# Jittor/InstanceSegmentation-jittor

Hardware: AMD Instinct MI355X
Metric: images/sec (Yolact R50-FPN 550x550, bs=8 per GPU, fp32) (higher is better)
Workload: dtype f32; 1 GPU; Yolact R50-FPN 550x550 bs=8/GPU random weights: uint8 upload + FastBaseTransform on the device + backbone+FPN+protonet+heads+Detect(fast-NMS)+550x550 mask assembly (BASELINE configs[1]); global_batch=8, parallelism=batch-sharded x1, RCCL all-gather of detections

## Files before the change

### include/isegmi.h

```cpp
#ifndef ISEGMI_H
#define ISEGMI_H
#include <stdint.h>
#ifdef __cplusplus
extern "C" {
#endif
#pragma GCC visibility push(default)

#define ISEGMI_ABI_VERSION 1

int isegmi_version(void);
const char* isegmi_last_error(void);

int isegmi_device_count(int* n);
int isegmi_set_device(int device_id);
int isegmi_malloc(void** d_ptr, int64_t bytes);
int isegmi_free(void* d_ptr);
int isegmi_malloc_host(void** h_ptr, int64_t bytes);
int isegmi_free_host(void* h_ptr);
int isegmi_h2d(void* d_dst, const void* h_src, int64_t bytes);
int isegmi_d2h(void* h_dst, const void* d_src, int64_t bytes);
int isegmi_memset(void* d_ptr, int value, int64_t bytes);
int isegmi_sync(void);
int isegmi_box_calibrate(double ms_per_leg, double* mfma_f32_tflops, double* mfma_f16_tflops, double* hbm_copy_gbs);

typedef struct isegmi_conv_desc {
    int32_t N, H, W, Cin;
    int32_t Cout, R, S, stride, pad;
    int32_t act;
    int32_t tile;
    int32_t out_div;
    int64_t out_img_stride;
    int64_t out_pix_stride;
} isegmi_conv_desc;

int isegmi_conv_out_hw(const isegmi_conv_desc* d, int32_t* Ho, int32_t* Wo);
int isegmi_conv_split_qualifies(const isegmi_conv_desc* d);
int isegmi_conv_packed_floats(const isegmi_conv_desc* d, int64_t* n);
int isegmi_pack_conv_weights(const isegmi_conv_desc* d, const float* h_w_krsc, float* h_packed);
int isegmi_op_conv2d(const isegmi_conv_desc* d, const float* d_in, const float* d_wpacked,
                     const float* d_scale, const float* d_shift, const float* d_residual,
                     float* d_out, void* stream);
int isegmi_op_conv2d_group(int n, const isegmi_conv_desc* descs, const float* const* d_in, const float* const* d_w, const float* const* d_scale,
                           const float* const* d_shift, const float* const* d_res, float* const* d_out, void* stream);

int isegmi_conv_grouped_packed_floats(const isegmi_conv_desc* d, int groups, int64_t* n);
int isegmi_pack_conv_weights_grouped(const isegmi_conv_desc* d, int groups, const float* h_w, float* h_packed);
int isegmi_op_conv2d_grouped(const isegmi_conv_desc* d, int groups, const float* d_in, const float* d_wpacked,
                             const float* d_scale, const float* d_shift, const float* d_residual,
                             float* d_out, void* stream);

int isegmi_conv_packed_halfs(const isegmi_conv_desc* d, int64_t* n);
int isegmi_pack_conv_weights_f16(const isegmi_conv_desc* d, const float* h_w_krsc, uint16_t* h_packed);
int isegmi_op_conv2d_f16(const isegmi_conv_desc* d, const void* d_in, const void* d_wpacked,
                         const float* d_scale, const float* d_shift, const void* d_residual, void* d_out,
                         int out_f32, void* stream);
typedef struct isegmi_bottleneck_desc {
    int32_t N, H, W, Cin, Cmid;
    int32_t flags;
} isegmi_bottleneck_desc;
int isegmi_op_bottleneck_f16(const isegmi_bottleneck_desc* d, const void* d_x, const void* d_w1, const float* d_s1, const float* d_b1,
                             const void* d_w2, const float* d_s2, const float* d_b2, const void* d_w3, const float* d_s3,
                             const float* d_b3, void* d_out, void* stream);
int isegmi_op_bottleneck_ds_f16(const isegmi_bottleneck_desc* d, const void* d_x, const void* d_w1, const float* d_s1, const float* d_b1,
                                const void* d_w2, const float* d_s2, const float* d_b2, const void* d_w3, const float* d_s3,
                                const float* d_b3, const void* d_wd, const float* d_sd, const float* d_bd, void* d_out, void* stream);
int isegmi_op_conv1x1_up2x_add_f16(const isegmi_conv_desc* d, const void* d_in, const void* d_wpacked, const float* d_scale, const float* d_shift,
                                   const void* d_coarse, int Hc, int Wc, void* d_out, void* stream);
int isegmi_op_conv3x3_head_f16(const isegmi_conv_desc* d, const void* d_in, const void* d_wpacked, const float* d_scale, const float* d_shift,
                               const void* d_w2packed, const float* d_scale2, const float* d_shift2, int cout2, float* d_out2, int* fused, void* stream);
int isegmi_op_pad_c3_to_f16_halo(const float* d_in_nhwc3, int N, int H, int W, void* d_out, void* stream);
int isegmi_op_stem_pool_f16(int N, int H, int W, const void* d_halo, const void* d_w, const float* d_scale, const float* d_shift, void* d_out,
                            int flags, void* stream);

int isegmi_set_f16_mfma_shape(int shape);
int isegmi_get_f16_mfma_shape(int* shape);

// ... 405 lines not shown
```

### instancesegmentation-jittor_amd/csrc/conv_mfma.hip

```cpp
#include <type_traits>
#include "../../include/isegmi.h"
#include "common.h"
#include "conv_korder.h"
#include "detmath.h"

#ifndef CONV_F32_RES_AUX
#define CONV_F32_RES_AUX 0
#endif

namespace isegmi {

typedef float f32x16 __attribute__((ext_vector_type(16)));

struct ConvK {
    const float* in;
    const float* w;
    const float* scale;
    const float* shift;
    const float* res;
    float* out;
    int N, H, W, Cin, Cout, R, S, stride, pad, Ho, Wo, M;
    int nchunks, cin_chunks;
    int kgroup;
    int64_t wrow;
// ... 221 lines not shown
                    acc[a][b] = __builtin_amdgcn_mfma_f32_32x32x2f32(fa[a].w, fb[b].w, acc[a][b], 0, 0, 0);
                }
        }
    };

    int cur = 0;
    for (int t = 0; t + 1 < p.nchunks; ++t) {
        load_chunk(t + 1);
        __builtin_amdgcn_sched_barrier(0);
        compute(cur);
        __builtin_amdgcn_sched_barrier(0);
        store_chunk(cur ^ 1);
        __syncthreads();
        cur ^= 1;
    }
    compute(cur);

#pragma unroll
    for (int a = 0; a < TM; ++a) {
#pragma unroll
        for (int b = 0; b < TN; ++b) {
            const int co = n0 + (wn * TN + b) * 32 + lr;
            const bool cok = co < p.Cout;
            const float sc = (cok && p.scale) ? p.scale[co] : 1.0f;
            const float sh = (cok && p.shift) ? p.shift[co] : 0.0f;
            Epi ep;
            epi_begin(p, m0 + (wm * TM + a) * 32 + 4 * lh, co, ep);
            epi_finish(p, acc[a][b], sc, sh, ep);
            __builtin_amdgcn_sched_barrier(0);
        }
    }
}

template <int RING, bool EARLY>
__device__ __forceinline__ void conv_v2_body(const ConvK& p, float* smem, const int bid, const int nwg) {
    constexpr int BM = 64, BN = 64;
    constexpr int STAGE = (BM + BN) * LDS_ROW;
    const int tid = threadIdx.x;
    const int lane = tid & 63, wave = __builtin_amdgcn_readfirstlane(tid >> 6);
    const int wm = wave >> 1, wn = wave & 1;
    const int q8 = nwg >> 3, r8 = nwg & 7, xcd = bid & 7;
    const int logical = (xcd < r8 ? xcd * (q8 + 1) : r8 * (q8 + 1) + (xcd - r8) * q8) + (bid >> 3);
    int mt, nt;
    conv_tile_of(p, logical, mt, nt);
    const int m0 = p.m_begin + mt * BM, n0 = nt * BN;

    const int lrow = tid >> 2, g = tid & 3;
    int hi0, wi0;
    unsigned abase;
    {
        const int m = m0 + lrow;
        if (m >= p.M) { hi0 = -(1 << 28); wi0 = 0; abase = 0; }
        else if (p.R * p.S == 1 && p.stride == 1 && p.pad == 0) {
            hi0 = 0; wi0 = 0;
            abase = ((unsigned)m * (unsigned)p.Cin + (unsigned)(g * 8)) * 4u;
        } else {
            const int hw = p.Ho * p.Wo;
            const int n = m / hw, rem = m - n * hw;
            const int ho = rem / p.Wo, wo = rem - ho * p.Wo;
            hi0 = ho * p.stride - p.pad; wi0 = wo * p.stride - p.pad;
            abase = ((unsigned)((n * p.H + hi0) * p.W + wi0) * (unsigned)p.Cin + (unsigned)(g * 8)) * 4u;
        }
    }
    const unsigned wbase = ((unsigned)(n0 + lrow) * (unsigned)p.wrow + (unsigned)(g * 8)) * 4u;
    constexpr unsigned OOB = 0x80000000u;
    typedef unsigned int u32x4 __attribute__((ext_vector_type(4)));
    auto make_rsrc = [](const void* ptr, unsigned bytes) {
        const unsigned long long a = (unsigned long long)ptr;
// ... 18 lines not shown
        asm volatile("buffer_load_dwordx4 %0, %1, %2, %3 offen" : "=v"(rb[slot][0]) : "v"(wbase), "s"(rsb), "s"(soffb) : "memory");
        asm volatile("buffer_load_dwordx4 %0, %1, %2, %3 offen offset:16" : "=v"(rb[slot][1]) : "v"(wbase), "s"(rsb), "s"(soffb) : "memory");
        ++chunk;
        soffa += 128u;
        if (conv_k_next(kr, ks, kc, kg, glen, p.R, p.S, p.kgroup, p.cin_chunks)) {
            soffa = (unsigned)kg * 128u;
            int tr = __builtin_amdgcn_readfirstlane(kr), ts = __builtin_amdgcn_readfirstlane(ks);
            asm volatile("" : "+s"(tr), "+s"(ts));
            const unsigned inb = (unsigned)((unsigned)(hi0 + tr) < (unsigned)p.H) & (unsigned)((unsigned)(wi0 + ts) < (unsigned)p.W);
            const unsigned tapv = abase + (unsigned)((tr * p.W + ts) * p.Cin) * 4u;
            avoff = inb ? tapv : OOB;
        }
    };
    typedef __attribute__((address_space(3))) void* lds_ptr;
    const unsigned lds_wr_addr = (unsigned)(uintptr_t)(lds_ptr)(smem + lrow * LDS_ROW + g * 8);
    auto store_chunk = [&](int slot, int stage, auto pending) {
        asm volatile("s_waitcnt vmcnt(%4)" : "+v"(ra[slot][0]), "+v"(ra[slot][1]), "+v"(rb[slot][0]), "+v"(rb[slot][1]) : "n"(decltype(pending)::value) : "memory");
        const unsigned wa = lds_wr_addr + (unsigned)(stage * STAGE * 4);
        asm volatile("ds_write2_b32 %0, %1, %2 offset1:1" :: "v"(wa), "v"(ra[slot][0].x), "v"(ra[slot][0].z) : "memory");
        asm volatile("ds_write2_b32 %0, %1, %2 offset0:2 offset1:3" :: "v"(wa), "v"(ra[slot][1].x), "v"(ra[slot][1].z) : "memory");
        asm volatile("ds_write2_b32 %0, %1, %2 offset0:4 offset1:5" :: "v"(wa), "v"(ra[slot][0].y), "v"(ra[slot][0].w) : "memory");
        asm volatile("ds_write2_b32 %0, %1, %2 offset0:6 offset1:7" :: "v"(wa), "v"(ra[slot][1].y), "v"(ra[slot][1].w) : "memory");
        asm volatile("ds_write_b128 %0, %1 offset:%2" :: "v"(wa), "v"(rb[slot][0]), "n"(BM * LDS_ROW * 4) : "memory");
        asm volatile("ds_write_b128 %0, %1 offset:%2" :: "v"(wa), "v"(rb[slot][1]), "n"(BM * LDS_ROW * 4 + 16) : "memory");
        asm volatile("s_waitcnt lgkmcnt(0)" ::: "memory");
    };

    f32x16 acc;
#pragma unroll
    for (int e = 0; e < 16; ++e) acc[e] = 0.0f;
    const int lr = lane & 31, lh = lane >> 5;
    const float* const lds_a = smem + (wm * 32 + lr) * LDS_ROW + lh * 4;
    const float* const lds_b = smem + BM * LDS_ROW + (wn * 32 + lr) * LDS_ROW + lh * 4;
    float4 fa[2], fb[2];
    auto read_frags = [&](int set, int stage, int gg) {
        fa[set] = *(const float4*)(lds_a + stage * STAGE + gg * 8);
        fb[set] = *(const float4*)(lds_b + stage * STAGE + gg * 8);
    };
    auto mma4 = [&](int set) {
        acc = __builtin_amdgcn_mfma_f32_32x32x2f32(fa[set].x, fb[set].x, acc, 0, 0, 0);
        acc = __builtin_amdgcn_mfma_f32_32x32x2f32(fa[set].y, fb[set].y, acc, 0, 0, 0);
        acc = __builtin_amdgcn_mfma_f32_32x32x2f32(fa[set].z, fb[set].z, acc, 0, 0, 0);
        acc = __builtin_amdgcn_mfma_f32_32x32x2f32(fa[set].w, fb[set].w, acc, 0, 0, 0);
    };
    auto compute = [&](int stage) {
#pragma unroll
        for (int gg = 0; gg < 4; ++gg) {
            if (gg < 3) read_frags((gg + 1) & 1, stage, gg + 1);
            mma4(gg & 1);
        }
    };
    typedef std::integral_constant<int, 4 * (RING - 1)> Steady;
    typedef std::integral_constant<int, 4 * (RING - 2) < 0 ? 0 : 4 * (RING - 2)> Early;
    static_assert(RING % 2 == 0, "the LDS stage of an unrolled position is its parity");

#pragma unroll
    for (int i = 0; i < RING; ++i) load_chunk(i);
    store_chunk(0, 0, Steady());
    __syncthreads();
    const int last = p.nchunks - 1;
    for (int t0 = 0; t0 < last; t0 += RING) {
#pragma unroll
        for (int j = 0; j < RING; ++j) {
            if (t0 + j >= last) break;
            const int cur = j & 1;
            read_frags(0, cur, 0);
            if (EARLY) store_chunk((j + 1) % RING, cur ^ 1, Early());
            load_chunk(j);
            __builtin_amdgcn_sched_barrier(0);
            compute(cur);
            __builtin_amdgcn_sched_barrier(0);
            if (!EARLY) store_chunk((j + 1) % RING, cur ^ 1, Steady());
            __syncthreads();
        }
    }
    const int cur = last & 1;
    const int co = n0 + wn * 32 + lr;
    const bool cok = co < p.Cout;
    Epi ep;
    epi_begin(p, m0 + wm * 32 + 4 * lh, co, ep);
    const float sc = (cok && p.scale) ? p.scale[co] : 1.0f;
    const float sh = (cok && p.shift) ? p.shift[co] : 0.0f;
    __builtin_amdgcn_sched_barrier(0);
    read_frags(0, cur, 0);
    compute(cur);
    __builtin_amdgcn_sched_barrier(0);
    asm volatile("s_waitcnt vmcnt(0)" ::: "memory");
#pragma unroll
    for (int i = 0; i < RING; ++i) asm volatile("" :: "v"(ra[i][0]), "v"(ra[i][1]), "v"(rb[i][0]), "v"(rb[i][1]));
    epi_finish(p, acc, sc, sh, ep);
}

template <int RING, bool EARLY>
__global__ __launch_bounds__(256, 4) void conv_mfma_v2_kernel(const ConvK p) {
    extern __shared__ __attribute__((aligned(16))) float smem[];
    conv_v2_body<RING, EARLY>(p, smem, (int)blockIdx.x, (int)gridDim.x);
}

typedef float f32x4 __attribute__((ext_vector_type(4)));

#ifndef EXPERIMENT_HALF_B
#define EXPERIMENT_HALF_B 0
#endif
#ifndef EXPERIMENT_NO_LOADS
#define EXPERIMENT_NO_LOADS 0
#endif
#ifndef EXPERIMENT_MODE
#define EXPERIMENT_MODE 0
#endif
template <int RING, bool LW, int WN = 1, int KS = 1>
__device__ __forceinline__ void conv_mfma16_body(const ConvK& p, float* smem16, const int bid, const int nwg) {
    static_assert(WN == 1 || !LW, "the loader-wave variant runs one tile per wave");
    static_assert(KS == 1 || (!LW && WN == 1), "split-K runs KS plain 32 x 32 sets");
    constexpr int BM = 32, BN = 32 * WN;
    constexpr int ROW = 34;
    constexpr int STAGE = (BM + BN) * ROW;
    constexpr int NST = LW ? 3 : 2;
    float* const smem_block = smem16;
    const int kset = KS > 1 ? __builtin_amdgcn_readfirstlane((int)(threadIdx.x >> 8)) : 0;
    if (KS > 1) smem16 += kset * NST * STAGE;
    const int count = KS > 1 ? (p.nchunks + KS - 1) / KS : p.nchunks;
    const int c_begin = KS > 1 ? min(kset * count, p.nchunks) : 0;
    const int c_end = KS > 1 ? min(c_begin + count, p.nchunks) : p.nchunks;

    const int tid = threadIdx.x & 255;
    const bool loader = LW && __builtin_amdgcn_readfirstlane((int)(threadIdx.x >> 8)) != 0;
    const int lane = tid & 63, wave = __builtin_amdgcn_readfirstlane(tid >> 6);
    const int wm = wave >> 1, wn = wave & 1;
    const int q8 = nwg >> 3, r8 = nwg & 7, xcd = bid & 7;
// ... 243 lines not shown
            for (int e = 0; e < 4; ++e) {
                float y = fmaf(acc[t][e], sc, sh);
                if (p.act == 4) {
                    y = y > 0.0f ? y : y * 0.1f;
                    yv[e] = y + rv[e];
                    continue;
                }
                y = y + rv[e];
                yv[e] = p.act == 3 ? (y > 0.0f ? y : y * 0.1f) : y;
            }
            if (p.act == 2) {
#pragma unroll
                for (int e = 0; e < 4; ++e) yv[e] = dm_tanh(yv[e]);
            }
        }
#pragma unroll
        for (int e = 0; e < 4; ++e) __builtin_amdgcn_raw_buffer_store_b32(__builtin_bit_cast(unsigned, yv[e]), rs_out, ooff[e], 0, 0);
    }
}

template <int RING, bool LW, int WN = 1>
__global__ __launch_bounds__(LW ? 512 : 256) void conv_mfma16_kernel(const ConvK p) {
    constexpr int STAGE16 = (32 + 32 * WN) * 34;
    __shared__ __attribute__((aligned(16))) float smem16[(LW ? 3 : 2) * STAGE16];
    conv_mfma16_body<RING, LW, WN>(p, smem16, (int)blockIdx.x, (int)gridDim.x);
}

template <int KS>
__global__ __launch_bounds__(256 * KS) void conv_mfma16_split_kernel(const ConvK p) {
    extern __shared__ __attribute__((aligned(16))) float smem_split[];
    conv_mfma16_body<4, false, 1, KS>(p, smem_split, (int)blockIdx.x, (int)gridDim.x);
}

template <int RING>
__global__ __launch_bounds__(256, 4) void conv_hybrid_kernel(const ConvK pm, const ConvK pt, const int nmain) {
    extern __shared__ __attribute__((aligned(16))) float smem[];
    if ((int)blockIdx.x < nmain) conv_v2_body<RING, false>(pm, smem, (int)blockIdx.x, nmain);
    else conv_mfma16_body<4, false, 1>(pt, smem, (int)blockIdx.x - nmain, (int)gridDim.x - nmain);
}

constexpr int CONV_GROUP_MAX = 10;
struct ConvGroupK {
    int n;
    int blk0[CONV_GROUP_MAX + 1];
    int kind[CONV_GROUP_MAX];
    ConvK k[CONV_GROUP_MAX];
};
static_assert(sizeof(ConvGroupK) <= 4096, "kernel arguments");
template <int RING>
__global__ __launch_bounds__(256, 4) void conv_group_kernel(const ConvGroupK g) {
    extern __shared__ __attribute__((aligned(16))) float smem[];
    int i = 0;
    while (i + 1 < g.n && (int)blockIdx.x >= g.blk0[i + 1]) ++i;
    const int bid = (int)blockIdx.x - g.blk0[i], nwg = g.blk0[i + 1] - g.blk0[i];
    if (g.kind[i] == 0) conv_v2_body<RING, false>(g.k[i], smem, bid, nwg);
    else conv_mfma16_body<4, false, 1>(g.k[i], smem, bid, nwg);
}

static bool is_stem(const isegmi_conv_desc* d) { return d->Cin == 4 && d->R == 7 && d->S == 7; }
static int cout_pad(const isegmi_conv_desc* d) { return cdiv(d->Cout, 128) * 128; }
static int n_chunks(const isegmi_conv_desc* d) { return is_stem(d) ? 7 : d->R * d->S * (d->Cin / 32); }

static int check_desc(const isegmi_conv_desc* d) {
    ARG_CHECK(d != nullptr, "null desc");
    ARG_CHECK(d->N > 0 && d->H > 0 && d->W > 0 && d->Cout > 0 && d->R > 0 && d->S > 0 && d->stride > 0 && d->pad >= 0,
              "non-positive conv geometry");
    ARG_CHECK(is_stem(d) || (d->Cin > 0 && d->Cin % 32 == 0), "Cin must be a multiple of 32 (or the Cin=4 7x7 stem)");
    ARG_CHECK(d->H + 2 * d->pad >= d->R && d->W + 2 * d->pad >= d->S, "kernel larger than padded input");
    ARG_CHECK(d->act >= 0 && d->act <= 4, "act");
    ARG_CHECK(d->tile >= 0 && d->tile <= 15, "tile");
    return ISEGMI_OK;
}

static void conv_set_band(ConvK& k, const int bn, const int blocks_per_cu, const int64_t in_touched) {
    static int legacy = -1;
    if (legacy < 0) { const char* e = getenv("ISEGMI_CONV_BAND"); legacy = (e && atoi(e) == 0) ? 1 : 0; }
    if (legacy) { k.nband = (int64_t)k.w_bytes > (int64_t)k.in_bytes ? 1 : k.ntiles; return; }
    const double A = (double)in_touched, B = (double)k.nchunks * 128.0 * bn * k.ntiles;
    const double l2_keep = 2.5e6;
    const double slots = 32.0 * blocks_per_cu;
    const double tiles_xcd = (double)k.mtiles * k.ntiles / 8.0;
    const double rounds = tiles_xcd / slots > 1.0 ? tiles_xcd / slots : 1.0;
    double best = 0;
    int best_bw = k.ntiles;
    for (int nb = 1; nb <= k.ntiles; nb *= 2) {
        const int bw = cdiv(k.ntiles, nb), nbands = cdiv(k.ntiles, bw);
        const double band_b = B / nbands;
        double a, b;
// ... 43 lines not shown
    k.in = in; k.w = w; k.scale = scale; k.shift = shift; k.res = res; k.out = out;
    k.N = d->N; k.H = d->H; k.W = d->W; k.Cin = d->Cin; k.Cout = d->Cout; k.R = d->R; k.S = d->S;
    k.stride = d->stride; k.pad = d->pad;
    k.Ho = (d->H + 2 * d->pad - d->R) / d->stride + 1;
    k.Wo = (d->W + 2 * d->pad - d->S) / d->stride + 1;
    const int64_t M64 = (int64_t)d->N * k.Ho * k.Wo;
    ARG_CHECK(M64 < (1ll << 31) - 256, "too many output pixels");
    k.M = (int)M64;
    k.nchunks = n_chunks(d);
    k.cin_chunks = is_stem(d) ? 1 : d->Cin / 32;
    k.kgroup = conv_kgroup(d->R, d->S, k.cin_chunks, is_stem(d));
    k.wrow = (int64_t)k.nchunks * 32;
    const int64_t in_bytes = (int64_t)d->N * d->H * d->W * d->Cin * 4;
    ARG_CHECK(in_bytes < (1ll << 31), "conv input must be < 2 GiB (32-bit buffer offsets)");
    k.in_bytes = (unsigned)in_bytes;
    k.w_bytes = (unsigned)((int64_t)cout_pad(d) * k.wrow * 4);
    k.in_touched = (d->R == 1 && d->S == 1 && d->stride > 1) ? in_bytes / ((int64_t)d->stride * d->stride) : in_bytes;
    k.m_begin = 0;
    k.act = d->act;
    k.out_div = d->out_div > 0 ? d->out_div : k.Ho * k.Wo;
    k.out_pix_stride = d->out_pix_stride > 0 ? d->out_pix_stride : d->Cout;
    k.out_img_stride = d->out_img_stride > 0 ? d->out_img_stride : (int64_t)k.out_div * k.out_pix_stride;
    k.contiguous = (k.out_img_stride == (int64_t)k.out_div * k.out_pix_stride) ? 1 : 0;
    const int64_t n_img = (k.M + k.out_div - 1) / k.out_div;
    const int64_t out_extent = ((n_img - 1) * k.out_img_stride + (int64_t)(k.out_div - 1) * k.out_pix_stride + d->Cout) * 4;
    ARG_CHECK(out_extent < (1ll << 31), "conv output span must be < 2 GiB (32-bit buffer offsets)");
    k.out_bytes = (unsigned)out_extent;
    k.res_bytes = (unsigned)((int64_t)k.M * d->Cout * 4);
    ARG_CHECK(res == nullptr || (int64_t)k.M * d->Cout * 4 < (1ll << 31), "residual must be < 2 GiB");
    k.mtiles = 0; k.ntiles = 0; k.nband = 0;
    return ISEGMI_OK;
}

static bool conv_hybrid_on() {
    static int on = -1;
    if (on < 0) { const char* e = getenv("ISEGMI_CONV_HYBRID"); on = (e && atoi(e) == 0) ? 0 : 1; }
    return on != 0;
}

int conv2d_launch(const isegmi_conv_desc* d, const float* in, const float* w, const float* scale, const float* shift,
                  const float* res, float* out, hipStream_t st) {
    ConvK k;
    const int rc_fill = conv_fill(d, in, w, scale, shift, res, out, k);
    if (rc_fill) return rc_fill;
    int tile = d->tile;
    if (tile == 0) {
        const int64_t t64 = (int64_t)cdiv(k.M, 64) * cdiv(d->Cout, 64);
        const int nck = k.nchunks;
        const int ncu = device_cu_count();
        const int v2 = nck >= 72 ? 12 : 10;
        if (is_stem(d)) tile = 3;
        else if (t64 <= 176) tile = 5;
        else if (nck <= 2 && d->Cout > 32) tile = v2;
        else if (d->Cout <= 32 || t64 <= 480) tile = 4;
        else if (t64 >= 513 && t64 % ncu != 0 && (t64 % ncu) * 100 <= t64 * 15 && conv_hybrid_on()) tile = 13;
        else if (t64 <= 512) tile = v2;
        else if (t64 <= 640) tile = nck >= 32 ? 6 : 4;
        else if (t64 <= 1024) tile = v2;
        else if (t64 <= 1100) tile = nck >= 32 ? 6 : 4;
        else tile = v2;
    }
    if (tile >= 4 && is_stem(d)) tile = 3;
    if (tile == 13 || tile == 14) {
        const int nt64 = cdiv(d->Cout, 64);
        const int64_t mt64 = cdiv(k.M, 64);
        const int ncu = device_cu_count();
        int64_t main_mt = (mt64 * nt64 / ncu) * ncu / nt64;
        if (main_mt * 64 > k.M) main_mt = k.M / 64;
        if (main_mt <= 0 || main_mt >= mt64) {
            tile = tile == 13 ? 10 : 12;
        } else {
            ConvK km = k, kt = k;
            km.mtiles = (int)main_mt; km.ntiles = nt64;
            kt.m_begin = (int)(main_mt * 64);
            kt.mtiles = cdiv(k.M - kt.m_begin, 32); kt.ntiles = cdiv(d->Cout, 32);
            const int64_t in_tail = (int64_t)((double)k.in_touched * (k.M - kt.m_begin) / k.M);
            conv_set_band(km, 64, 4, k.in_touched - in_tail);
            conv_set_band(kt, 32, 4, in_tail);
            const int nmain = km.mtiles * km.ntiles, ntail = kt.mtiles * kt.ntiles;
            const size_t lds = 2 * (size_t)(64 + 64) * LDS_ROW * sizeof(float);
            if (tile == 13) hipLaunchKernelGGL((conv_hybrid_kernel<2>), dim3((unsigned)(nmain + ntail)), dim3(256), lds, st, km, kt, nmain);
            else hipLaunchKernelGGL((conv_hybrid_kernel<4>), dim3((unsigned)(nmain + ntail)), dim3(256), lds, st, km, kt, nmain);
            HIP_TRY(hipGetLastError());
            return ISEGMI_OK;
        }
    }
    if (tile == 15) {
        ARG_CHECK(!is_stem(d), "split-K: not for the stem");
        constexpr int KS = 4;
        k.mtiles = cdiv(k.M, 32);
        k.ntiles = cdiv(d->Cout, 32);
        conv_set_band(k, 32, 1, k.in_touched);
        const size_t lds = (size_t)KS * 2 * (32 + 32) * 34 * sizeof(float);
        LDS_LIMIT_ONCE((int)lds, conv_mfma16_split_kernel<KS>);
        hipLaunchKernelGGL((conv_mfma16_split_kernel<KS>), dim3((unsigned)(k.mtiles * k.ntiles)), dim3(256 * KS), lds, st, k);
        HIP_TRY(hipGetLastError());
        return ISEGMI_OK;
    }
    if (tile >= 7) {
        ARG_CHECK(tile != 8 && tile != 11, "tiles 8 / 11 (ring of 3) were dropped: the LDS stage of an unrolled position is its parity");
        k.mtiles = cdiv(k.M, 64);
        k.ntiles = cdiv(d->Cout, 64);
        const size_t lds = 2 * (size_t)(64 + 64) * LDS_ROW * sizeof(float);
        conv_set_band(k, 64, 4, k.in_touched);
        const dim3 g7((unsigned)(k.mtiles * k.ntiles));
        if (tile == 7) hipLaunchKernelGGL((conv_mfma_v2_kernel<2, true>), g7, dim3(256), lds, st, k);
        else if (tile == 9) hipLaunchKernelGGL((conv_mfma_v2_kernel<4, true>), g7, dim3(256), lds, st, k);
        else if (tile == 10) hipLaunchKernelGGL((conv_mfma_v2_kernel<2, false>), g7, dim3(256), lds, st, k);
        else hipLaunchKernelGGL((conv_mfma_v2_kernel<4, false>), g7, dim3(256), lds, st, k);
        HIP_TRY(hipGetLastError());
        return ISEGMI_OK;
    }
    if (tile >= 4) {
        k.mtiles = cdiv(k.M, 32);
        k.ntiles = cdiv(d->Cout, tile == 6 ? 64 : 32);
        conv_set_band(k, tile == 6 ? 64 : 32, tile == 4 ? 8 : 4, k.in_touched);
        const dim3 g16((unsigned)(k.mtiles * k.ntiles));
        if (tile == 5) hipLaunchKernelGGL((conv_mfma16_kernel<8, true>), g16, dim3(512), 0, st, k);
        else if (tile == 6) hipLaunchKernelGGL((conv_mfma16_kernel<4, false, 2>), g16, dim3(256), 0, st, k);
        else hipLaunchKernelGGL((conv_mfma16_kernel<4, false>), g16, dim3(256), 0, st, k);
        HIP_TRY(hipGetLastError());
        return ISEGMI_OK;
    }
    switch (tile) {
        case 1: return launch<128, 128, 2, 2>(d, k, st);
        case 2: return launch<128, 64, 2, 2>(d, k, st);
        default: return launch<64, 64, 2, 2>(d, k, st);
    }
}

int conv2d_group_launch(int n, const isegmi_conv_desc* const* d, const float* const* in, const float* const* w, const float* const* scale,
                        const float* const* shift, const float* const* res, float* const* out, hipStream_t st) {
    ARG_CHECK(n >= 1 && n <= CONV_GROUP_MAX && d && in && w && out, "conv group: 1..10 members");
    ConvGroupK g;
    ConvK ks[CONV_GROUP_MAX];
    int64_t t64[CONV_GROUP_MAX], total64 = 0;
    for (int i = 0; i < n; ++i) {
        ARG_CHECK(d[i] && !is_stem(d[i]) && d[i]->tile == 0, "conv group: no stem, no forced tile");
        ARG_CHECK(in[i] && w[i] && out[i], "conv group: a member's input, weights or output pointer is NULL");
        const int rc = conv_fill(d[i], in[i], w[i], scale ? scale[i] : nullptr, shift ? shift[i] : nullptr, res ? res[i] : nullptr, out[i], ks[i]);
        if (rc) return rc;
        t64[i] = (int64_t)cdiv(ks[i].M, 64) * cdiv(d[i]->Cout, 64);
        total64 += t64[i];
    }
    int order[CONV_GROUP_MAX], kind[CONV_GROUP_MAX];
    int ring = 2;
    for (int i = 0; i < n; ++i) {
        order[i] = i;
        kind[i] = (total64 > 480 && t64[i] >= 256 && d[i]->Cout > 32) ? 0 : 1;
        if (kind[i] == 0 && ks[i].nchunks >= 72) ring = 4;
    }
    for (int a = 1; a < n; ++a)
        for (int b = a; b > 0; --b) {
            const int x = order[b - 1], y = order[b];
            const bool swap = kind[y] < kind[x] || (kind[y] == kind[x] && t64[y] > t64[x]);
            if (!swap) break;
            order[b - 1] = y; order[b] = x;
        }
    g.n = n;
    g.blk0[0] = 0;
    for (int j = 0; j < n; ++j) {
        const int i = order[j];
        ConvK& k = ks[i];
        const int bt = kind[i] == 0 ? 64 : 32;
        k.mtiles = cdiv(k.M, bt);
        k.ntiles = cdiv(d[i]->Cout, bt);
        conv_set_band(k, bt, kind[i] == 0 ? 4 : 8, k.in_touched);
        const int64_t blocks = (int64_t)k.mtiles * k.ntiles;
        ARG_CHECK(g.blk0[j] + blocks < (1ll << 30), "conv group: too many tiles");
        g.k[j] = k;
        g.kind[j] = kind[i];
        g.blk0[j + 1] = g.blk0[j] + (int)blocks;
    }
    const size_t lds = 2 * (size_t)(64 + 64) * LDS_ROW * sizeof(float);
    if (ring == 4) hipLaunchKernelGGL((conv_group_kernel<4>), dim3((unsigned)g.blk0[n]), dim3(256), lds, st, g);
    else hipLaunchKernelGGL((conv_group_kernel<2>), dim3((unsigned)g.blk0[n]), dim3(256), lds, st, g);
    HIP_TRY(hipGetLastError());
    return ISEGMI_OK;
}

}

using namespace isegmi;

extern "C" int isegmi_op_conv2d_group(int n, const isegmi_conv_desc* descs, const float* const* d_in, const float* const* d_w, const float* const* d_scale,
                                      const float* const* d_shift, const float* const* d_res, float* const* d_out, void* stream) {
    ARG_CHECK(n >= 1 && n <= CONV_GROUP_MAX && descs, "conv group: 1..10 members");
    const isegmi_conv_desc* dp[CONV_GROUP_MAX];
    for (int i = 0; i < n; ++i) dp[i] = descs + i;
    return conv2d_group_launch(n, dp, d_in, d_w, d_scale, d_shift, d_res, d_out, (hipStream_t)stream);
}

extern "C" int isegmi_conv_split_qualifies(const isegmi_conv_desc* d) {
    if (!d || check_desc(d) != ISEGMI_OK || is_stem(d)) return 0;
    const int Ho = (d->H + 2 * d->pad - d->R) / d->stride + 1, Wo = (d->W + 2 * d->pad - d->S) / d->stride + 1;
    const int64_t M = (int64_t)d->N * Ho * Wo;
    const int64_t t64 = ((M + 63) / 64) * ((d->Cout + 63) / 64);
    return t64 <= 176 && n_chunks(d) >= 32 ? 1 : 0;
}

extern "C" int isegmi_conv_out_hw(const isegmi_conv_desc* d, int32_t* Ho, int32_t* Wo) {
    int rc = check_desc(d);
    if (rc) return rc;
    *Ho = (d->H + 2 * d->pad - d->R) / d->stride + 1;
    *Wo = (d->W + 2 * d->pad - d->S) / d->stride + 1;
    return ISEGMI_OK;
}

extern "C" int isegmi_conv_packed_floats(const isegmi_conv_desc* d, int64_t* n) {
    int rc = check_desc(d);
    if (rc) return rc;
    *n = (int64_t)cout_pad(d) * n_chunks(d) * 32;
    return ISEGMI_OK;
}

extern "C" int isegmi_pack_conv_weights(const isegmi_conv_desc* d, const float* w, float* packed) {
    int rc = check_desc(d);
    if (rc) return rc;
    ARG_CHECK(w && packed, "null pointer");
    const int nch = n_chunks(d);
    const int64_t wrow = (int64_t)nch * 32;
    const int64_t total = (int64_t)cout_pad(d) * wrow;
    for (int64_t i = 0; i < total; ++i) packed[i] = 0.0f;
    const int K = d->R * d->S * d->Cin;
    for (int co = 0; co < d->Cout; ++co) {
        const float* src = w + (int64_t)co * K;
        float* dst = packed + (int64_t)co * wrow;
        if (is_stem(d)) {
            for (int r = 0; r < 7; ++r)
                for (int e = 0; e < 28; ++e) {
                    const int grp = e >> 3, pos = conv_perm8(e & 7);
// ... 15 lines not shown
```

### instancesegmentation-jittor_amd/isegmi/_abi.py

```python
import ctypes as C

RETINA_MAX_LEVELS = 5


def _i32(*names):
    return [(n, C.c_int32) for n in names]


def _ptr(*names):
    return [(n, C.c_void_p) for n in names]


class ConvDesc(C.Structure):
    _fields_ = _i32("N", "H", "W", "Cin", "Cout", "R", "S", "stride", "pad", "act", "tile", "out_div") + \
        [("out_img_stride", C.c_int64), ("out_pix_stride", C.c_int64)]


class BottleneckDesc(C.Structure):
    _fields_ = _i32("N", "H", "W", "Cin", "Cmid", "flags")


class YolactDetectArgs(C.Structure):
    _fields_ = _i32("N", "P", "ncls", "mask_dim", "top_k", "max_det") + [("conf_thresh", C.c_float), ("nms_thresh", C.c_float)] + \
        _ptr("d_conf", "d_loc", "d_mask", "d_priors", "d_ws_scoresT", "d_ws_boxes", "d_ws_counts", "d_ws_tk_vals", "d_ws_tk_idx", "d_ws_tk_cnt",
# ... 39 lines not shown

class CocoMatchArgs(C.Structure):
    _fields_ = _i32("n_groups", "A", "T", "reserved") + [("n_dets", C.c_int64), ("n_gts", C.c_int64), ("n_ious", C.c_int64)] + \
        _ptr("d_det_off", "d_gt_off", "d_iou_off", "d_ious", "d_det_area", "d_gt_area", "d_gt_crowd", "d_gt_ignore", "d_area_rng", "d_iou_thrs",
             "d_dt_match", "d_dt_ignore", "d_gt_match", "d_gt_ignore_out")


STRUCTS = {"isegmi_conv_desc": ConvDesc, "isegmi_bottleneck_desc": BottleneckDesc, "isegmi_yolact_detect_args": YolactDetectArgs,
           "isegmi_box_post_args": BoxPostArgs, "isegmi_retina_select_args": RetinaSelectArgs, "isegmi_retina_post_args": RetinaPostArgs,
           "isegmi_rle_args": RleArgs, "isegmi_p2s_image": P2sImage, "isegmi_coco_match_args": CocoMatchArgs}

I, L, F, D, S, V = C.c_int, C.c_int64, C.c_float, C.c_double, C.c_char_p, C.c_void_p

SIGNATURES = {
    "isegmi_version": (I, []),
    "isegmi_last_error": (S, []),
    "isegmi_device_count": (I, [V]),
    "isegmi_set_device": (I, [I]),
    "isegmi_malloc": (I, [V, L]),
    "isegmi_free": (I, [V]),
    "isegmi_malloc_host": (I, [V, L]),
    "isegmi_free_host": (I, [V]),
    "isegmi_h2d": (I, [V, V, L]),
    "isegmi_d2h": (I, [V, V, L]),
    "isegmi_memset": (I, [V, I, L]),
    "isegmi_sync": (I, []),
    "isegmi_box_calibrate": (I, [D, V, V, V]),
    "isegmi_conv_out_hw": (I, [V, V, V]),
    "isegmi_conv_split_qualifies": (I, [V]),
    "isegmi_conv_packed_floats": (I, [V, V]),
    "isegmi_pack_conv_weights": (I, [V, V, V]),
    "isegmi_op_conv2d": (I, [V, V, V, V, V, V, V, V]),
    "isegmi_op_conv2d_group": (I, [I, V, V, V, V, V, V, V, V]),
    "isegmi_conv_grouped_packed_floats": (I, [V, I, V]),
    "isegmi_pack_conv_weights_grouped": (I, [V, I, V, V]),
    "isegmi_op_conv2d_grouped": (I, [V, I, V, V, V, V, V, V, V]),
    "isegmi_conv_packed_halfs": (I, [V, V]),
    "isegmi_pack_conv_weights_f16": (I, [V, V, V]),
    "isegmi_op_conv2d_f16": (I, [V, V, V, V, V, V, V, I, V]),
    "isegmi_op_bottleneck_f16": (I, [V, V, V, V, V, V, V, V, V, V, V, V, V]),
    "isegmi_op_bottleneck_ds_f16": (I, [V, V, V, V, V, V, V, V, V, V, V, V, V, V, V, V]),
    "isegmi_op_conv1x1_up2x_add_f16": (I, [V, V, V, V, V, V, I, I, V, V]),
    "isegmi_op_conv3x3_head_f16": (I, [V, V, V, V, V, V, V, V, I, V, V, V]),
    "isegmi_op_pad_c3_to_f16_halo": (I, [V, I, I, I, V, V]),
    "isegmi_op_stem_pool_f16": (I, [I, I, I, V, V, V, V, V, I, V]),
    "isegmi_set_f16_mfma_shape": (I, [I]),
    "isegmi_get_f16_mfma_shape": (I, [V]),
    "isegmi_op_preprocess_u8": (I, [V, I, I, I, V, I, I, I, I, L, V, V, I, V]),
    "isegmi_op_preprocess_u8_flip": (I, [V, I, I, I, V, I, I, I, I, L, V, V, I, I, V]),
    "isegmi_resample_coeffs": (I, [I, I, V, V, V]),
    "isegmi_op_resample_u8": (I, [V, L, V, V, I, V, L, V, I, I, I, L, V, V, I, F, V, L, V]),
    "isegmi_op_resample_tile": (I, [V, V, V]),
    "isegmi_op_maxpool": (I, [V, I, I, I, I, I, I, I, V, V]),
    "isegmi_op_resize_bilinear": (I, [V, I, I, I, I, I, I, V, I, V, V]),
    "isegmi_op_keypoint_heatmap": (I, [V, L, I, I, I, V, V]),
    "isegmi_op_keypoint_decode": (I, [V, V, V, I, I, I, I, V, V, V]),
    "isegmi_op_deform_im2col": (I, [V, I, I, I, I, V, I, I, I, I, I, V, V]),
    "isegmi_op_deform_im2col_v1": (I, [V, I, I, I, I, V, I, I, I, I, I, V, V]),
    "isegmi_op_deform_conv2d": (I, [V, I, I, I, I, V, I, I, I, V, I, V, V, V, I, V, V]),
    "isegmi_op_upsample_nearest2x_add": (I, [V, I, I, I, I, V, I, I, V, V]),
    "isegmi_op_group_norm_workspace_bytes": (L, [L, I, I, I, I]),
    "isegmi_op_group_norm": (I, [V, L, I, I, I, I, V, V, F, V, I, V, V, L, V]),
    "isegmi_op_pad_c3_to_c4": (I, [V, L, V, V]),
    "isegmi_op_map_f32": (I, [V, V, L, I, V]),
    "isegmi_op_maxpool_f16": (I, [V, I, I, I, I, I, I, I, I, V, V]),
    "isegmi_op_resize_bilinear_f16": (I, [V, I, I, I, I, I, I, V, I, V, V]),
# ... 136 lines not shown
```

Before: 1032 img/s.

## Add software-pipelined MFMA schedule to fp32 conv v2 kernel

Adds a new V2_SCHED form of the fp32 MFMA conv body. It hand-interleaves LDS fragment reads, LDS stores of the next chunk, global loads and the chunk barrier between individual MFMA instructions, using explicit waitcnt and sched_barrier. The goal is to hide LDS and global latency behind MFMA issue rather than running the store and compute phases back to back. It is on by default for convs with at least 16 K-chunks and can be disabled through an environment variable or an API override. The cost is more fragile hand-scheduled asm, with tail handling that risks correctness or register pressure.

```diff
diff --git a/include/isegmi.h b/include/isegmi.h
--- a/include/isegmi.h
+++ b/include/isegmi.h
@@ -42,6 +42,7 @@
                      float* d_out, void* stream);
 int isegmi_op_conv2d_group(int n, const isegmi_conv_desc* descs, const float* const* d_in, const float* const* d_w, const float* const* d_scale,
                            const float* const* d_shift, const float* const* d_res, float* const* d_out, void* stream);
+int isegmi_conv_sched_override(int mode);
 
 int isegmi_conv_grouped_packed_floats(const isegmi_conv_desc* d, int groups, int64_t* n);
 int isegmi_pack_conv_weights_grouped(const isegmi_conv_desc* d, int groups, const float* h_w, float* h_packed);
diff --git a/instancesegmentation-jittor_amd/csrc/conv_mfma.hip b/instancesegmentation-jittor_amd/csrc/conv_mfma.hip
--- a/instancesegmentation-jittor_amd/csrc/conv_mfma.hip
+++ b/instancesegmentation-jittor_amd/csrc/conv_mfma.hip
@@ -277,8 +277,27 @@
     }
 }
 
-template <int RING, bool EARLY>
+#ifndef EXPERIMENT_V2_MODE
+#define EXPERIMENT_V2_MODE 0
+#endif
+#ifndef CONV_SCHED_BARRIER_AT
+#define CONV_SCHED_BARRIER_AT 12
+#endif
+#ifndef CONV_SCHED_STORE_AT
+#define CONV_SCHED_STORE_AT 0
+#endif
+static_assert(CONV_SCHED_BARRIER_AT == 12 || (CONV_SCHED_BARRIER_AT == 8 && CONV_SCHED_STORE_AT == 0), "the writes end in front of the chunk barrier");
+static_assert(CONV_SCHED_STORE_AT == 0 || CONV_SCHED_STORE_AT == 4, "writes behind MFMA 0-6 or 4-10");
+enum { V2_LATE = 0, V2_EARLY = 1, V2_SCHED = 2 };
+constexpr int conv_sched_write_at(const int k) { return CONV_SCHED_STORE_AT + (k < 5 ? k : 6); }
+constexpr int conv_sched_writes(const int lo, const int hi) {
+    int n = 0;
+    for (int k = 0; k < 6; ++k) n += (conv_sched_write_at(k) >= lo && conv_sched_write_at(k) < hi) ? 1 : 0;
+    return n;
+}
+template <int RING, int FORM>
 __device__ __forceinline__ void conv_v2_body(const ConvK& p, float* smem, const int bid, const int nwg) {
+    constexpr bool EARLY = FORM == V2_EARLY;
     constexpr int BM = 64, BN = 64;
     constexpr int STAGE = (BM + BN) * LDS_ROW;
     const int tid = threadIdx.x;
@@ -363,10 +382,11 @@
     const int lr = lane & 31, lh = lane >> 5;
     const float* const lds_a = smem + (wm * 32 + lr) * LDS_ROW + lh * 4;
     const float* const lds_b = smem + BM * LDS_ROW + (wn * 32 + lr) * LDS_ROW + lh * 4;
-    float4 fa[2], fb[2];
+    typedef float frag4 __attribute__((ext_vector_type(4)));
+    frag4 fa[2], fb[2];
     auto read_frags = [&](int set, int stage, int gg) {
-        fa[set] = *(const float4*)(lds_a + stage * STAGE + gg * 8);
-        fb[set] = *(const float4*)(lds_b + stage * STAGE + gg * 8);
+        fa[set] = *(const frag4*)(lds_a + stage * STAGE + gg * 8);
+        fb[set] = *(const frag4*)(lds_b + stage * STAGE + gg * 8);
     };
     auto mma4 = [&](int set) {
         acc = __builtin_amdgcn_mfma_f32_32x32x2f32(fa[set].x, fb[set].x, acc, 0, 0, 0);
@@ -384,48 +404,189 @@
     typedef std::integral_constant<int, 4 * (RING - 1)> Steady;
     typedef std::integral_constant<int, 4 * (RING - 2) < 0 ? 0 : 4 * (RING - 2)> Early;
     static_assert(RING % 2 == 0, "the LDS stage of an unrolled position is its parity");
-
-#pragma unroll
-    for (int i = 0; i < RING; ++i) load_chunk(i);
-    store_chunk(0, 0, Steady());
-    __syncthreads();
-    const int last = p.nchunks - 1;
-    for (int t0 = 0; t0 < last; t0 += RING) {
-#pragma unroll
-        for (int j = 0; j < RING; ++j) {
-            if (t0 + j >= last) break;
-            const int cur = j & 1;
-            read_frags(0, cur, 0);
-            if (EARLY) store_chunk((j + 1) % RING, cur ^ 1, Early());
-            load_chunk(j);
-            __builtin_amdgcn_sched_barrier(0);
-            compute(cur);
-            __builtin_amdgcn_sched_barrier(0);
-            if (!EARLY) store_chunk((j + 1) % RING, cur ^ 1, Steady());
-            __syncthreads();
-        }
-    }
-    const int cur = last & 1;
+    constexpr bool NO_BARRIER = (EXPERIMENT_V2_MODE & 1) != 0, NO_STORES = (EXPERIMENT_V2_MODE & 2) != 0;
+
     const int co = n0 + wn * 32 + lr;
     const bool cok = co < p.Cout;
     Epi ep;
-    epi_begin(p, m0 + wm * 32 + 4 * lh, co, ep);
-    const float sc = (cok && p.scale) ? p.scale[co] : 1.0f;
-    const float sh = (cok && p.shift) ? p.shift[co] : 0.0f;
-    __builtin_amdgcn_sched_barrier(0);
-    read_frags(0, cur, 0);
-    compute(cur);
-    __builtin_amdgcn_sched_barrier(0);
-    asm volatile("s_waitcnt vmcnt(0)" ::: "memory");
-#pragma unroll
-    for (int i = 0; i < RING; ++i) asm volatile("" :: "v"(ra[i][0]), "v"(ra[i][1]), "v"(rb[i][0]), "v"(rb[i][1]));
+    float sc, sh;
+    const int last = p.nchunks - 1;
+
+    if constexpr (FORM == V2_SCHED) {
+        const unsigned ra_addr = (unsigned)(uintptr_t)(lds_ptr)lds_a, rb_addr = (unsigned)(uintptr_t)(lds_ptr)lds_b;
+        auto frag_read = [&](auto SET, auto STG, auto GG) {
+            constexpr int set = decltype(SET)::value, off = decltype(STG)::value * STAGE * 4 + decltype(GG)::value * 32;
+            asm volatile("ds_read_b128 %0, %1 offset:%2" : "=v"(fa[set]) : "v"(ra_addr), "n"(off) : "memory");
+            asm volatile("ds_read_b128 %0, %1 offset:%2" : "=v"(fb[set]) : "v"(rb_addr), "n"(off) : "memory");
+            __builtin_amdgcn_sched_barrier(0);
+        };
+        auto frag_wait = [&](auto SET, auto PENDING) {
+            constexpr int set = decltype(SET)::value;
+            asm volatile("s_waitcnt lgkmcnt(%2)" : "+v"(fa[set]), "+v"(fb[set]) : "n"(decltype(PENDING)::value) : "memory");
+            __builtin_amdgcn_sched_barrier(0);
+        };
+        auto mf = [&](float a, float b) {
+            acc = __builtin_amdgcn_mfma_f32_32x32x2f32(a, b, acc, 0, 0, 0);
+            __builtin_amdgcn_sched_barrier(0);
+        };
+        typedef std::integral_constant<int, 0> I0;
+        typedef std::integral_constant<int, 1> I1;
+        typedef std::integral_constant<int, 2> I2;
+        typedef std::integral_constant<int, 3> I3;
+        constexpr int NW = NO_STORES ? 0 : 1;
+        auto chunk_barrier = [&]() {
+            asm volatile("s_waitcnt lgkmcnt(0)" : "+v"(fa[1]), "+v"(fb[1]) :: "memory");
+            if (!NO_BARRIER) __builtin_amdgcn_s_barrier();
+            __builtin_amdgcn_sched_barrier(0);
+        };
+        auto sched_iter = [&](auto JC, auto TAIL) {
+            constexpr int j = decltype(JC)::value, slot = (j + 1) % RING;
+            constexpr bool tail = decltype(TAIL)::value != 0;
+            typedef std::integral_constant<int, j & 1> Cur;
+            typedef std::integral_constant<int, (j & 1) ^ 1> Nxt;
+            const unsigned wa = lds_wr_addr + (unsigned)(Nxt::value * STAGE * 4);
+            auto write = [&](auto KC) {
+                constexpr int k = decltype(KC)::value;
+                if constexpr (k == 0) asm volatile("ds_write2_b32 %0, %1, %2 offset1:1" :: "v"(wa), "v"(ra[slot][0].x), "v"(ra[slot][0].z) : "memory");
+                if constexpr (k == 1) asm volatile("ds_write2_b32 %0, %1, %2 offset0:2 offset1:3" :: "v"(wa), "v"(ra[slot][1].x), "v"(ra[slot][1].z) : "memory");
+                if constexpr (k == 2) asm volatile("ds_write2_b32 %0, %1, %2 offset0:4 offset1:5" :: "v"(wa), "v"(ra[slot][0].y), "v"(ra[slot][0].w) : "memory");
+                if constexpr (k == 3) asm volatile("ds_write2_b32 %0, %1, %2 offset0:6 offset1:7" :: "v"(wa), "v"(ra[slot][1].y), "v"(ra[slot][1].w) : "memory");
+                if constexpr (k == 4) asm volatile("ds_write_b128 %0, %1 offset:%2" :: "v"(wa), "v"(rb[slot][0]), "n"(BM * LDS_ROW * 4) : "memory");
+                if constexpr (k == 5) asm volatile("ds_write_b128 %0, %1 offset:%2" :: "v"(wa), "v"(rb[slot][1]), "n"(BM * LDS_ROW * 4 + 16) : "memory");
+                __builtin_amdgcn_sched_barrier(0);
+            };
+            auto mfw = [&](auto IDX, float a, float b) {
+                constexpr int idx = decltype(IDX)::value;
+                if constexpr (idx == conv_sched_write_at(0) && !NO_STORES && !tail) {
+                    asm volatile("s_waitcnt vmcnt(%4)" : "+v"(ra[slot][0]), "+v"(ra[slot][1]), "+v"(rb[slot][0]), "+v"(rb[slot][1]) : "n"(4 * (RING - 1)) : "memory");
+                    __builtin_amdgcn_sched_barrier(0);
+                }
+                mf(a, b);
+                if constexpr (!NO_STORES) {
+                    if constexpr (idx == conv_sched_write_at(0)) write(I0());
+                    if constexpr (idx == conv_sched_write_at(1)) write(I1());
+                    if constexpr (idx == conv_sched_write_at(2)) write(I2());
+                    if constexpr (idx == conv_sched_write_at(3)) write(I3());
+                    if constexpr (idx == conv_sched_write_at(4)) write(std::integral_constant<int, 4>());
+                    if constexpr (idx == conv_sched_write_at(5)) write(std::integral_constant<int, 5>());
+                }
+            };
+            typedef std::integral_constant<int, 4> I4;
+            typedef std::integral_constant<int, 5> I5;
+            typedef std::integral_constant<int, 6> I6;
+            typedef std::integral_constant<int, 7> I7;
+            __builtin_amdgcn_sched_barrier(0);
+            frag_read(I1(), Cur(), I1());
+            frag_wait(I0(), I2());
+            mfw(I0(), fa[0].x, fb[0].x);
+            mfw(I1(), fa[0].y, fb[0].y);
+            mfw(I2(), fa[0].z, fb[0].z);
+            mfw(I3(), fa[0].w, fb[0].w);
+            frag_read(I0(), Cur(), I2());
+            frag_wait(I1(), std::integral_constant<int, NW * conv_sched_writes(0, 4) + 2>());
+            mfw(I4(), fa[1].x, fb[1].x);
+            mfw(I5(), fa[1].y, fb[1].y);
+            mfw(I6(), fa[1].z, fb[1].z);
+            mfw(I7(), fa[1].w, fb[1].w);
+            frag_read(I1(), Cur(), I3());
+            frag_wait(I0(), std::integral_constant<int, NW * conv_sched_writes(4, 8) + 2>());
+            if (CONV_SCHED_BARRIER_AT == 8) chunk_barrier();
+            mfw(std::integral_constant<int, 8>(), fa[0].x, fb[0].x);
+            mfw(std::integral_constant<int, 9>(), fa[0].y, fb[0].y);
+            mfw(std::integral_constant<int, 10>(), fa[0].z, fb[0].z);
+            mfw(std::integral_constant<int, 11>(), fa[0].w, fb[0].w);
+            if (CONV_SCHED_BARRIER_AT != 8) chunk_barrier();
+            frag_read(I0(), Nxt(), I0());
+            if constexpr (!tail) load_chunk(slot);
+            __builtin_amdgcn_sched_barrier(0);
+            mf(fa[1].x, fb[1].x);
+            mf(fa[1].y, fb[1].y);
+            mf(fa[1].z, fb[1].z);
+            mf(fa[1].w, fb[1].w);
+        };
+#pragma unroll
+        for (int i = 0; i < RING; ++i) load_chunk(i);
+        store_chunk(0, 0, Steady());
+        __builtin_amdgcn_s_barrier();
+        __builtin_amdgcn_sched_barrier(0);
+        frag_read(I0(), I0(), I0());
+        load_chunk(0);
+        __builtin_amdgcn_sched_barrier(0);
+        const int rounds = last / RING, rem = last - rounds * RING;
+        for (int r = 0; r < rounds; ++r) {
+            sched_iter(I0(), I0());
+            sched_iter(I1(), I0());
+            if constexpr (RING == 4) {
+                sched_iter(I2(), I0());
+                sched_iter(I3(), I0());
+            }
+        }
+        asm volatile("s_waitcnt vmcnt(0)" ::: "memory");
+#pragma unroll
+        for (int i = 0; i < RING; ++i) asm volatile("" : "+v"(ra[i][0]), "+v"(ra[i][1]), "+v"(rb[i][0]), "+v"(rb[i][1]));
+        __builtin_amdgcn_sched_barrier(0);
+        frag_wait(I0(), I0());
+        if (rem >= 1) { sched_iter(I0(), I1()); frag_wait(I0(), I0()); }
+        if constexpr (RING == 4) {
+            if (rem >= 2) { sched_iter(I1(), I1()); frag_wait(I0(), I0()); }
+            if (rem >= 3) { sched_iter(I2(), I1()); frag_wait(I0(), I0()); }
+        }
+        epi_begin(p, m0 + wm * 32 + 4 * lh, co, ep);
+        sc = (cok && p.scale) ? p.scale[co] : 1.0f;
+        sh = (cok && p.shift) ? p.shift[co] : 0.0f;
+        __builtin_amdgcn_sched_barrier(0);
+        auto last_chunk = [&](auto CUR) {
+            frag_read(I1(), CUR, I1());
+            mf(fa[0].x, fb[0].x); mf(fa[0].y, fb[0].y); mf(fa[0].z, fb[0].z); mf(fa[0].w, fb[0].w);
+            frag_read(I0(), CUR, I2());
+            frag_wait(I1(), I2());
+            mf(fa[1].x, fb[1].x); mf(fa[1].y, fb[1].y); mf(fa[1].z, fb[1].z); mf(fa[1].w, fb[1].w);
+            frag_read(I1(), CUR, I3());
+            frag_wait(I0(), I2());
+            mf(fa[0].x, fb[0].x); mf(fa[0].y, fb[0].y); mf(fa[0].z, fb[0].z); mf(fa[0].w, fb[0].w);
+            frag_wait(I1(), I0());
+            mf(fa[1].x, fb[1].x); mf(fa[1].y, fb[1].y); mf(fa[1].z, fb[1].z); mf(fa[1].w, fb[1].w);
+        };
+        if (last & 1) last_chunk(I1()); else last_chunk(I0());
+    } else {
+#pragma unroll
+        for (int i = 0; i < RING; ++i) load_chunk(i);
+        store_chunk(0, 0, Steady());
+        __syncthreads();
+        for (int t0 = 0; t0 < last; t0 += RING) {
+#pragma unroll
+            for (int j = 0; j < RING; ++j) {
+                if (t0 + j >= last) break;
+                const int cur = j & 1;
+                read_frags(0, cur, 0);
+                if (EARLY && !NO_STORES) store_chunk((j + 1) % RING, cur ^ 1, Early());
+                load_chunk(j);
+                __builtin_amdgcn_sched_barrier(0);
+                compute(cur);
+                __builtin_amdgcn_sched_barrier(0);
+                if (!EARLY && !NO_STORES) store_chunk((j + 1) % RING, cur ^ 1, Steady());
+                if (!NO_BARRIER) __syncthreads();
+            }
+        }
+        const int cur = last & 1;
+        epi_begin(p, m0 + wm * 32 + 4 * lh, co, ep);
+        sc = (cok && p.scale) ? p.scale[co] : 1.0f;
+        sh = (cok && p.shift) ? p.shift[co] : 0.0f;
+        __builtin_amdgcn_sched_barrier(0);
+        read_frags(0, cur, 0);
+        compute(cur);
+        __builtin_amdgcn_sched_barrier(0);
+        asm volatile("s_waitcnt vmcnt(0)" ::: "memory");
+#pragma unroll
+        for (int i = 0; i < RING; ++i) asm volatile("" :: "v"(ra[i][0]), "v"(ra[i][1]), "v"(rb[i][0]), "v"(rb[i][1]));
+    }
     epi_finish(p, acc, sc, sh, ep);
 }
 
-template <int RING, bool EARLY>
+template <int RING, int FORM>
 __global__ __launch_bounds__(256, 4) void conv_mfma_v2_kernel(const ConvK p) {
     extern __shared__ __attribute__((aligned(16))) float smem[];
-    conv_v2_body<RING, EARLY>(p, smem, (int)blockIdx.x, (int)gridDim.x);
+    conv_v2_body<RING, FORM>(p, smem, (int)blockIdx.x, (int)gridDim.x);
 }
 
 typedef float f32x4 __attribute__((ext_vector_type(4)));
@@ -735,10 +896,10 @@
     conv_mfma16_body<4, false, 1, KS>(p, smem_split, (int)blockIdx.x, (int)gridDim.x);
 }
 
-template <int RING>
+template <int RING, int FORM>
 __global__ __launch_bounds__(256, 4) void conv_hybrid_kernel(const ConvK pm, const ConvK pt, const int nmain) {
     extern __shared__ __attribute__((aligned(16))) float smem[];
-    if ((int)blockIdx.x < nmain) conv_v2_body<RING, false>(pm, smem, (int)blockIdx.x, nmain);
+    if ((int)blockIdx.x < nmain) conv_v2_body<RING, FORM>(pm, smem, (int)blockIdx.x, nmain);
     else conv_mfma16_body<4, false, 1>(pt, smem, (int)blockIdx.x - nmain, (int)gridDim.x - nmain);
 }
 
@@ -750,13 +911,13 @@
     ConvK k[CONV_GROUP_MAX];
 };
 static_assert(sizeof(ConvGroupK) <= 4096, "kernel arguments");
-template <int RING>
+template <int RING, int FORM>
 __global__ __launch_bounds__(256, 4) void conv_group_kernel(const ConvGroupK g) {
     extern __shared__ __attribute__((aligned(16))) float smem[];
     int i = 0;
     while (i + 1 < g.n && (int)blockIdx.x >= g.blk0[i + 1]) ++i;
     const int bid = (int)blockIdx.x - g.blk0[i], nwg = g.blk0[i + 1] - g.blk0[i];
-    if (g.kind[i] == 0) conv_v2_body<RING, false>(g.k[i], smem, bid, nwg);
+    if (g.kind[i] == 0) conv_v2_body<RING, FORM>(g.k[i], smem, bid, nwg);
     else conv_mfma16_body<4, false, 1>(g.k[i], smem, bid, nwg);
 }
 
@@ -866,6 +1027,15 @@
     return ISEGMI_OK;
 }
 
+constexpr int CONV_SCHED_MIN_CHUNKS = 16;
+static int g_conv_sched_override = -1;
+static bool conv_sched_on(const int nchunks) {
+    static int env = -1;
+    if (env < 0) { const char* e = getenv("ISEGMI_CONV_SCHED"); env = (e && atoi(e) == 0) ? 0 : 1; }
+    if (g_conv_sched_override >= 0) return g_conv_sched_override != 0;
+    return env != 0 && nchunks >= CONV_SCHED_MIN_CHUNKS;
+}
+
 static bool conv_hybrid_on() {
     static int on = -1;
     if (on < 0) { const char* e = getenv("ISEGMI_CONV_HYBRID"); on = (e && atoi(e) == 0) ? 0 : 1; }
@@ -913,8 +1083,14 @@
             conv_set_band(kt, 32, 4, in_tail);
             const int nmain = km.mtiles * km.ntiles, ntail = kt.mtiles * kt.ntiles;
             const size_t lds = 2 * (size_t)(64 + 64) * LDS_ROW * sizeof(float);
-            if (tile == 13) hipLaunchKernelGGL((conv_hybrid_kernel<2>), dim3((unsigned)(nmain + ntail)), dim3(256), lds, st, km, kt, nmain);
-            else hipLaunchKernelGGL((conv_hybrid_kernel<4>), dim3((unsigned)(nmain + ntail)), dim3(256), lds, st, km, kt, nmain);
+            const dim3 gh((unsigned)(nmain + ntail));
+            if (conv_sched_on(k.nchunks)) {
+                if (tile == 13) hipLaunchKernelGGL((conv_hybrid_kernel<2, V2_SCHED>), gh, dim3(256), lds, st, km, kt, nmain);
+                else hipLaunchKernelGGL((conv_hybrid_kernel<4, V2_SCHED>), gh, dim3(256), lds, st, km, kt, nmain);
+            } else {
+                if (tile == 13) hipLaunchKernelGGL((conv_hybrid_kernel<2, V2_LATE>), gh, dim3(256), lds, st, km, kt, nmain);
+                else hipLaunchKernelGGL((conv_hybrid_kernel<4, V2_LATE>), gh, dim3(256), lds, st, km, kt, nmain);
+            }
             HIP_TRY(hipGetLastError());
             return ISEGMI_OK;
         }
@@ -938,10 +1114,13 @@
         const size_t lds = 2 * (size_t)(64 + 64) * LDS_ROW * sizeof(float);
         conv_set_band(k, 64, 4, k.in_touched);
         const dim3 g7((unsigned)(k.mtiles * k.ntiles));
-        if (tile == 7) hipLaunchKernelGGL((conv_mfma_v2_kernel<2, true>), g7, dim3(256), lds, st, k);
-        else if (tile == 9) hipLaunchKernelGGL((conv_mfma_v2_kernel<4, true>), g7, dim3(256), lds, st, k);
-        else if (tile == 10) hipLaunchKernelGGL((conv_mfma_v2_kernel<2, false>), g7, dim3(256), lds, st, k);
-        else hipLaunchKernelGGL((conv_mfma_v2_kernel<4, false>), g7, dim3(256), lds, st, k);
+        if (conv_sched_on(k.nchunks)) {
+            if (tile == 7 || tile == 10) hipLaunchKernelGGL((conv_mfma_v2_kernel<2, V2_SCHED>), g7, dim3(256), lds, st, k);
+            else hipLaunchKernelGGL((conv_mfma_v2_kernel<4, V2_SCHED>), g7, dim3(256), lds, st, k);
+        } else if (tile == 7) hipLaunchKernelGGL((conv_mfma_v2_kernel<2, V2_EARLY>), g7, dim3(256), lds, st, k);
+        else if (tile == 9) hipLaunchKernelGGL((conv_mfma_v2_kernel<4, V2_EARLY>), g7, dim3(256), lds, st, k);
+        else if (tile == 10) hipLaunchKernelGGL((conv_mfma_v2_kernel<2, V2_LATE>), g7, dim3(256), lds, st, k);
+        else hipLaunchKernelGGL((conv_mfma_v2_kernel<4, V2_LATE>), g7, dim3(256), lds, st, k);
         HIP_TRY(hipGetLastError());
         return ISEGMI_OK;
     }
@@ -978,11 +1157,12 @@
         total64 += t64[i];
     }
     int order[CONV_GROUP_MAX], kind[CONV_GROUP_MAX];
-    int ring = 2;
+    int ring = 2, nck64 = 0;
     for (int i = 0; i < n; ++i) {
         order[i] = i;
         kind[i] = (total64 > 480 && t64[i] >= 256 && d[i]->Cout > 32) ? 0 : 1;
         if (kind[i] == 0 && ks[i].nchunks >= 72) ring = 4;
+        if (kind[i] == 0 && ks[i].nchunks > nck64) nck64 = ks[i].nchunks;
     }
     for (int a = 1; a < n; ++a)
         for (int b = a; b > 0; --b) {
@@ -1007,8 +1187,14 @@
         g.blk0[j + 1] = g.blk0[j] + (int)blocks;
     }
     const size_t lds = 2 * (size_t)(64 + 64) * LDS_ROW * sizeof(float);
-    if (ring == 4) hipLaunchKernelGGL((conv_group_kernel<4>), dim3((unsigned)g.blk0[n]), dim3(256), lds, st, g);
-    else hipLaunchKernelGGL((conv_group_kernel<2>), dim3((unsigned)g.blk0[n]), dim3(256), lds, st, g);
+    const dim3 gg((unsigned)g.blk0[n]);
+    if (conv_sched_on(nck64)) {
+        if (ring == 4) hipLaunchKernelGGL((conv_group_kernel<4, V2_SCHED>), gg, dim3(256), lds, st, g);
+        else hipLaunchKernelGGL((conv_group_kernel<2, V2_SCHED>), gg, dim3(256), lds, st, g);
+    } else {
+        if (ring == 4) hipLaunchKernelGGL((conv_group_kernel<4, V2_LATE>), gg, dim3(256), lds, st, g);
+        else hipLaunchKernelGGL((conv_group_kernel<2, V2_LATE>), gg, dim3(256), lds, st, g);
+    }
     HIP_TRY(hipGetLastError());
     return ISEGMI_OK;
 }
@@ -1031,6 +1217,12 @@
     const int64_t M = (int64_t)d->N * Ho * Wo;
     const int64_t t64 = ((M + 63) / 64) * ((d->Cout + 63) / 64);
     return t64 <= 176 && n_chunks(d) >= 32 ? 1 : 0;
+}
+
+extern "C" int isegmi_conv_sched_override(int mode) {
+    ARG_CHECK(mode >= -1 && mode <= 1, "conv sched override: -1 (environment), 0 (previous schedule) or 1 (software-pipelined)");
+    g_conv_sched_override = mode;
+    return ISEGMI_OK;
 }
 
 extern "C" int isegmi_conv_out_hw(const isegmi_conv_desc* d, int32_t* Ho, int32_t* Wo) {
diff --git a/instancesegmentation-jittor_amd/isegmi/_abi.py b/instancesegmentation-jittor_amd/isegmi/_abi.py
--- a/instancesegmentation-jittor_amd/isegmi/_abi.py
+++ b/instancesegmentation-jittor_amd/isegmi/_abi.py
@@ -95,6 +95,7 @@
     "isegmi_pack_conv_weights": (I, [V, V, V]),
     "isegmi_op_conv2d": (I, [V, V, V, V, V, V, V, V]),
     "isegmi_op_conv2d_group": (I, [I, V, V, V, V, V, V, V, V]),
+    "isegmi_conv_sched_override": (I, [I]),
     "isegmi_conv_grouped_packed_floats": (I, [V, I, V]),
     "isegmi_pack_conv_weights_grouped": (I, [V, I, V, V]),
     "isegmi_op_conv2d_grouped": (I, [V, I, V, V, V, V, V, V, V]),
```

Result: no change. 1040 img/s (median of 6 runs) (+0.8%).
